# vyasakash231/gaussian_process_transportation

Measured on AMD Instinct MI355X. Metric: posterior (mean+var+Jacobian) preds/sec, N=8192 source pts, 3-D fp64, higher is better.
Workload: dtype f64; 1 GPU; N=8192 source pts, M=500000 queries per GPU per step, D=O=3, mean+var+Jacobian, RBF GP, fp64; queries_per_gpu=500000, mode=J

## Files before the change

gaussian_process_transportation_amd/csrc/gpt_kvar_i8.h:

```cpp
#pragma once
#include "gpt_common.h"
#include "gpt_dispatch.h"
#include "gpt_exp.h"
#include "gpt_plan_i8.h"

namespace gpt {

typedef int v4i __attribute__((ext_vector_type(4)));

constexpr int I8_TILE_STEPS = I8_ROWS / I8_KSTEP;
constexpr size_t I8_A_STEP = (size_t)8 * 4 * 64;
constexpr size_t I8_B_STEP = (size_t)8 * 64;
constexpr size_t I8_CHUNK = I8_TILE_STEPS * I8_B_STEP;
constexpr size_t I8_LDS_BYTES = 2 * I8_CHUNK * sizeof(v4i);
constexpr size_t I8_PARK_WORDS = var_i8_park_bytes() / 4;

#ifndef GPT_ABL_I8
#define GPT_ABL_I8 0
#endif
constexpr bool I8_ABL_A = GPT_ABL_I8 == 1 || GPT_ABL_I8 == 3 || GPT_ABL_I8 == 6;
constexpr bool I8_ABL_B = GPT_ABL_I8 == 2 || GPT_ABL_I8 == 3 || GPT_ABL_I8 == 6;
constexpr bool I8_ABL_NOGEN = GPT_ABL_I8 == 4;
constexpr bool I8_ABL_NORED = GPT_ABL_I8 == 5;
constexpr bool I8_ABL_NOLDS = GPT_ABL_I8 == 6;

struct I8Tab {
    float m[I8_NMOD], rm[I8_NMOD];
    float inv[I8_NMOD];
    float w[I8_NMOD][I8_NMOD];
};
constexpr int i8_balanced(int x, int m) { x %= m; if (x < 0) x += m; return x > (m - 1) / 2 ? x - m : x; }
constexpr I8Tab make_i8_tab() {
    I8Tab t{};
    for (int i = 0; i < I8_NMOD; ++i) {
        const int m = I8_MODULI[i];
        t.m[i] = (float)m; t.rm[i] = 1.0f / (float)m;
        int prod = 1;
        for (int l = 0; l < I8_NMOD; ++l) {
            t.w[l][i] = l < i ? (float)i8_balanced(prod, m) : 0.0f;
            if (l < i) prod = prod * I8_MODULI[l] % m;
        }
        int inv = 0;
        for (int x = 1; x < m; ++x) if (prod * x % m == 1) inv = x;
        t.inv[i] = (float)i8_balanced(inv, m);
    }
    return t;
}
static constexpr I8Tab I8_TAB = make_i8_tab();

__constant__ double c_i8_mod[I8_NMOD] = {256, 255, 253, 251, 247, 241, 239, 233, 229, 227, 223, 217, 211, 199};
__constant__ double c_i8_inv[I8_NMOD] = {1.0 / 256, 1.0 / 255, 1.0 / 253, 1.0 / 251, 1.0 / 247, 1.0 / 241, 1.0 / 239,
                                         1.0 / 233, 1.0 / 229, 1.0 / 227, 1.0 / 223, 1.0 / 217, 1.0 / 211, 1.0 / 199};
__constant__ double c_i8_hi[I8_NMOD] = {127, 127, 126, 125, 123, 120, 119, 116, 114, 113, 111, 108, 105, 99};
__constant__ double c_i8_lo[I8_NMOD] = {-128, -127, -126, -125, -123, -120, -119, -116, -114, -113, -111, -108, -105, -99};

static __device__ __forceinline__ int i8_residue(const double x, const double m, const double inv, const double hi, const double lo) {
    const double q = rint(x * inv);
    double r = fma(-q, m, x);
    r = r > hi ? r - m : r;
    r = r < lo ? r + m : r;
    return (int)r;
}
static __device__ __forceinline__ int i8_pack4(const int r0, const int r1, const int r2, const int r3) {
    return (int)((unsigned)(r0 & 255) | ((unsigned)(r1 & 255) << 8) | ((unsigned)(r2 & 255) << 16) | ((unsigned)r3 << 24));
}
static __device__ __forceinline__ void i8_store_planes(const double (&x)[16], v4i* __restrict__ dst, const size_t stride) {
#pragma unroll 1
    for (int j = 0; j < I8_NMOD; ++j) {
        const double m = c_i8_mod[j], inv = c_i8_inv[j], hi = c_i8_hi[j], lo = c_i8_lo[j];
        int r[16];
#pragma unroll
        for (int b = 0; b < 16; ++b) r[b] = i8_residue(x[b], m, inv, hi, lo);
        v4i o;
#pragma unroll
        for (int v = 0; v < 4; ++v) o[v] = i8_pack4(r[4 * v], r[4 * v + 1], r[4 * v + 2], r[4 * v + 3]);
        dst[(size_t)j * stride] = o;
    }
}

__global__ __launch_bounds__(256) void k_i8_rowmax(const double* __restrict__ Wf, unsigned long long* __restrict__ rowmax) {
    const int tile = blockIdx.x, g = blockIdx.y, th = threadIdx.x;
    int ib = 0;
    while ((ib + 1) * (ib + 2) / 2 <= tile) ++ib;
    const double* src = Wf + (size_t)tile * WT_TILE_DOUBLES + (size_t)g * 256 + th;
    double mx = 0.0;
    for (int k4 = 0; k4 < WT_K4; ++k4) mx = fmax(mx, fabs(src[(size_t)k4 * WT_STEP_DOUBLES]));
    const int q = th >> 7, lane = (th >> 1) & 63, pp = th & 1;
    const int row = ib * WT + 64 * g + 16 * (2 * q + pp) + (lane & 15);
    if (mx > 0.0) atomicMax(rowmax + row, (unsigned long long)__double_as_longlong(mx));
}
__global__ __launch_bounds__(256) void k_i8_rowscale(const unsigned long long* __restrict__ rowmax, int NP, int p, double* __restrict__ rowscale,
                                                     double* __restrict__ qscale) {
    const int i = blockIdx.x * 256 + threadIdx.x;
    if (i >= NP) return;
    const double mx = __longlong_as_double((long long)rowmax[i]);
    int e = 0;
    if (mx > 0.0) {
        int ex;
        const double f = frexp(mx, &ex);
        e = f == 0.5 ? ex - 1 : ex;
    }
    rowscale[i] = ldexp(1.0, e - p);
    qscale[i] = ldexp(1.0, p - e);
}
__global__ __launch_bounds__(256) void k_i8_planes(const double* __restrict__ Wf, const double* __restrict__ qscale, int ntiles, v4i* __restrict__ planes) {
    const int tile = blockIdx.x, g = blockIdx.y;
    int ib = 0;
    while ((ib + 1) * (ib + 2) / 2 <= tile) ++ib;
    const double* src = Wf + (size_t)tile * WT_TILE_DOUBLES;
    for (int u = threadIdx.x; u < I8_TILE_STEPS * 4 * 64; u += 256) {
        const int lane = u & 63, r = (u >> 6) & 3, s = u >> 8;
        const int lr = lane & 15, lk = lane >> 4;
        const double sc = qscale[ib * WT + 64 * g + 16 * r + lr];
        double x[16];
#pragma unroll
        for (int b = 0; b < 16; ++b) {
            const int col = 64 * s + 16 * lk + b;
            const int k4 = col >> 2, lkk = col & 3;
            x[b] = rint(src[((((size_t)k4 * 8 + g) * 2 + (r >> 1)) * 64 + lkk * 16 + lr) * 2 + (r & 1)] * sc);
        }
        v4i* dst = planes + ((((size_t)tile * I8_TILE_STEPS + s) * 8 + g) * 4 + r) * 64 + lane;
        i8_store_planes(x, dst, (size_t)ntiles * I8_TILE_STEPS * I8_A_STEP);
    }
}

static __device__ __forceinline__ double i8_garner(const float (&r)[I8_NMOD]) {
    float d[I8_NMOD];
    d[0] = r[0];
#pragma unroll
    for (int i = 1; i < I8_NMOD; ++i) {
        float s = 0.0f;
#pragma unroll
        for (int l = 0; l < i; ++l) s = fmaf(d[l], I8_TAB.w[l][i], s);
        float u = r[i] - s;
        u = fmaf(-rintf(u * I8_TAB.rm[i]), I8_TAB.m[i], u);
        const float v = u * I8_TAB.inv[i];
        d[i] = fmaf(-rintf(v * I8_TAB.rm[i]), I8_TAB.m[i], v);
    }
    double X = (double)d[I8_NMOD - 1];
#pragma unroll
    for (int i = I8_NMOD - 2; i >= 0; --i) X = fma(X, (double)I8_TAB.m[i], (double)d[i]);
    return X;
}

struct VarI8Args {
    const v4i* planes;
    const double* rowscale;
    const double* Xs;
    const double* Xq;
    int64_t M;
    double* slab;
    v4i* bimg;
    unsigned* park;
    double bq;
    double colscale;
    int ntiles;
};

template <int KT>
__global__ __launch_bounds__(512, 2) void k_var_i8(KernelParams p, VarI8PlanDev pl, VarI8Args a) {
    extern __shared__ __attribute__((aligned(16))) unsigned char i8_lds_raw[];
    v4i* const Bs = reinterpret_cast<v4i*>(i8_lds_raw);
    __shared__ double red[8][I8_COLS];
    __shared__ double Tt[256];
    const int tid = threadIdx.x, lane = tid & 63;
    const int w = __builtin_amdgcn_readfirstlane(tid >> 6);
    const int lc = lane & 15, lk = lane >> 4;
    const int g = (w < 4) ? w : (11 - w);
    const int nbi = pl.nbi, D = p.D;
    const int nst = p.NP / I8_KSTEP;
    if (tid < 256) Tt[tid] = g_exp2_table[tid];
    v4i* const bim = a.bimg + (size_t)blockIdx.x * ((size_t)I8_NMOD * nst * I8_B_STEP);
    unsigned* const pk = a.park + (size_t)blockIdx.x * I8_PARK_WORDS + tid;
    const size_t a_plane = (size_t)a.ntiles * I8_TILE_STEPS * I8_A_STEP;
    const v4i* const a_group = a.planes + (size_t)g * 256;
    const unsigned ulane = lane, utid = tid;
    constexpr double RS2 = 0.70710678118654752440;
    const double lnc = p.lnc;
    const int64_t n_rounds = pl.rnd_end - pl.rnd_begin;

    for (int64_t it = 0;; ++it) {
        int64_t cb; int ib_lo, ib_hi;
        if (it < n_rounds) {
            cb = (pl.rnd_begin + it) * pl.P + blockIdx.x; ib_lo = 0; ib_hi = nbi;
        } else {
            if (it > n_rounds || !pl.with_tail || pl.nparts <= 0) break;
            const int64_t c = blockIdx.x / pl.nparts;
            if (c >= pl.ncb - pl.nfull) break;
            const int q = blockIdx.x % pl.nparts;
            cb = pl.nfull + c; ib_lo = pl.bounds[q]; ib_hi = pl.bounds[q + 1];
        }
        __syncthreads();
        __builtin_amdgcn_fence(__ATOMIC_ACQ_REL, "workgroup");
        {
            const int64_t col = cb * I8_COLS + 16 * w + lc;
            const int64_t mm = col < a.M ? col : a.M - 1;
            const double* qp = a.Xq + mm * D;
            double q[3];
#pragma unroll
            for (int d = 0; d < 3; ++d) q[d] = qp[d < D ? d : 0] * ((d < D) ? p.inv_ls[d] * 0.70710678118654752440 : 0.0);
#pragma unroll 1
            for (int s = 0; s < (I8_ABL_NOGEN ? 0 : I8_TILE_STEPS * ib_hi); ++s) {
                const double* xp = a.Xs + (size_t)(I8_KSTEP * s + 16 * lk) * 4;
                double x[16];
#pragma unroll
                for (int b = 0; b < 16; ++b) {
                    const d4 xs = *reinterpret_cast<const d4*>(xp + 4 * b);
                    const double d0 = xs[0] * RS2 - q[0], d1 = xs[1] * RS2 - q[1], d2_ = xs[2] * RS2 - q[2];
                    double hh = d0 * d0;
                    hh = fma(d1, d1, hh);
                    hh = fma(d2_, d2_, hh);
                    x[b] = rint(kernel_tab<KT>(hh, lnc, Tt) * a.bq);
                }
                i8_store_planes(x, bim + ((size_t)s * 8 + w) * 64 + lane, (size_t)nst * I8_B_STEP);
            }
        }
        asm volatile("s_waitcnt vmcnt(0)" ::: "memory");
        __syncthreads();

        for (int ib = ib_hi - 1; ib >= ib_lo; --ib) {
            const int nmine = (g + 2) & ~1;
            const int lim = I8_TILE_STEPS * ib + nmine;
            const size_t tile0 = (size_t)ib * (ib + 1) / 2;
            auto a_ptr = [&](int j, int S) -> const v4i* {
                if (S >= lim) { S -= lim; ++j; }
                if (S >= lim) { S -= lim; ++j; }
                if (j >= I8_NMOD) { j = I8_NMOD - 1; S = lim - 1; }
                if (I8_ABL_A) S &= I8_TILE_STEPS - 1;
                return a_group + (size_t)j * a_plane + (tile0 * I8_TILE_STEPS + S) * I8_A_STEP;
            };
            {
                v4i t8[8];
#pragma unroll
                for (int i = 0; i < 8; ++i) t8[i] = bim[utid + 512 * i];
#pragma unroll
                for (int i = 0; i < 8; ++i) Bs[tid + 512 * i] = t8[i];
            }
            v4i ar[4][4];
#pragma unroll
            for (int i = 0; i < 4; ++i) {
                const v4i* ap = a_ptr(0, i);
#pragma unroll
                for (int r = 0; r < 4; ++r) ar[i][r] = ap[ulane + 64 * r];
            }
            __syncthreads();
            v4i acc[4][8];
#pragma unroll
            for (int r = 0; r < 4; ++r)
#pragma unroll
                for (int t = 0; t < 8; ++t) acc[r][t] = v4i{0, 0, 0, 0};
            int buf = 0;
            auto tile = [&](auto full_tag, const int nrun, const bool more_rt, const int j, const int S0, const v4i* nsrc) __attribute__((always_inline)) {
                constexpr bool FULL = decltype(full_tag)::value;
                const bool more = FULL || more_rt;
                if (I8_ABL_B) nsrc = bim;
                const v4i* bcur = Bs + (size_t)buf * I8_CHUNK + lane;
                v4i* bnext = Bs + (size_t)(buf ^ 1) * I8_CHUNK + tid;
                v4i st[3];
                v4i bq[3];
                if (I8_ABL_NOLDS) bq[0] = bq[1] = bq[2] = bcur[0];
#pragma unroll
                for (int s = 0; s < I8_TILE_STEPS; ++s) {
                    const bool run = FULL || s < nrun;
                    if (more && s == 0) st[0] = nsrc[utid];
                    if (more && s + 1 < I8_TILE_STEPS) st[(s + 1) % 3] = nsrc[utid + 512 * (s + 1)];
                    __builtin_amdgcn_sched_barrier(0);
                    if (run) {
                        if (!I8_ABL_NOLDS && (s == 0 || !FULL)) {
                            bq[(8 * s) % 3] = bcur[(8 * s) * 64];
                            bq[(8 * s + 1) % 3] = bcur[(8 * s + 1) * 64];
                        }
#pragma unroll
                        for (int t = 0; t < 8; ++t) {
                            const int u = 8 * s + t;
                            if (!I8_ABL_NOLDS && (t + 2 < 8 || (FULL && s + 1 < I8_TILE_STEPS))) bq[(u + 2) % 3] = bcur[(u + 2) * 64];
                            __builtin_amdgcn_sched_barrier(0);
#pragma unroll
                            for (int r = 0; r < 4; ++r)
                                acc[r][t] = __builtin_amdgcn_mfma_i32_16x16x64_i8(ar[s & 3][r], bq[u % 3], acc[r][t], 0, 0, 0);
                            __builtin_amdgcn_sched_barrier(0);
                        }
                    }
                    __builtin_amdgcn_sched_barrier(0);
                    if (more && s > 0) bnext[512 * (s - 1)] = st[(s - 1) % 3];
                    if (run) {
                        const v4i* ap = a_ptr(j, S0 + s + 4);
#pragma unroll
                        for (int r = 0; r < 4; ++r) ar[s & 3][r] = ap[ulane + 64 * r];
                    }
                    __builtin_amdgcn_sched_barrier(0);
                }
                if (more) bnext[512 * (I8_TILE_STEPS - 1)] = st[(I8_TILE_STEPS - 1) % 3];
                __syncthreads();
                buf ^= 1;
            };
#pragma unroll 1
            for (int j = 0; j < I8_NMOD; ++j) {
#pragma unroll 1
                for (int kb = 0; kb < ib; ++kb)
                    tile(Bool<true>{}, I8_TILE_STEPS, true, j, kb * I8_TILE_STEPS, bim + ((size_t)j * nst + (kb + 1) * I8_TILE_STEPS) * I8_B_STEP);
                tile(Bool<false>{}, nmine, j + 1 < I8_NMOD, j, ib * I8_TILE_STEPS, bim + (size_t)(j + 1) * nst * I8_B_STEP);
                if (I8_ABL_NORED) {
#pragma unroll
                    for (int r = 0; r < 4; ++r)
#pragma unroll
                        for (int t = 0; t < 8; ++t) asm volatile("" : "+v"(acc[r][t]));
                } else {
                    const double m = c_i8_mod[j], inv = c_i8_inv[j], hi = c_i8_hi[j], lo = c_i8_lo[j];
#pragma unroll
                    for (int r = 0; r < 4; ++r)
#pragma unroll
                        for (int t = 0; t < 8; ++t) {
                            int rr[4];
#pragma unroll
                            for (int e = 0; e < 4; ++e) rr[e] = i8_residue((double)acc[r][t][e], m, inv, hi, lo);
                            pk[(size_t)(j * 32 + r * 8 + t) * 512] = (unsigned)i8_pack4(rr[0], rr[1], rr[2], rr[3]);
                            acc[r][t] = v4i{0, 0, 0, 0};
                        }
                }
                const bool turn = (nmine & 2) != 0;
#pragma unroll
                for (int i = 0; i < 2; ++i)
#pragma unroll
                    for (int r = 0; r < 4; ++r) {
                        const v4i lo2 = ar[i][r], hi2 = ar[i + 2][r];
                        ar[i][r] = turn ? hi2 : lo2;
                        ar[i + 2][r] = turn ? lo2 : hi2;
                    }
            }
            asm volatile("s_waitcnt vmcnt(0)" ::: "memory");
#pragma unroll 1
            for (int t = 0; t < 8; ++t) {
                double ssq = 0.0;
#pragma unroll 1
                for (int r = 0; r < (I8_ABL_NORED ? 0 : 4); ++r) {
                    unsigned wd[I8_NMOD];
#pragma unroll
                    for (int j = 0; j < I8_NMOD; ++j) wd[j] = pk[(size_t)(j * 32 + r * 8 + t) * 512];
                    const d4 rs = *reinterpret_cast<const d4*>(a.rowscale + (size_t)ib * I8_ROWS + 64 * g + 16 * r + 4 * lk);
#pragma unroll
                    for (int e = 0; e < 4; ++e) {
                        float res[I8_NMOD];
#pragma unroll
                        for (int j = 0; j < I8_NMOD; ++j) res[j] = (float)((int)(wd[j] << (24 - 8 * e)) >> 24);
                        const double v = i8_garner(res) * rs[e] * a.colscale;
                        ssq = fma(v, v, ssq);
                    }
                }
                ssq += __shfl_xor(ssq, 16);
                ssq += __shfl_xor(ssq, 32);
                if (lk == 0) red[w][16 * t + lc] = ssq;
            }
            __syncthreads();
            if (tid < I8_COLS) {
                double v = 0.0;
#pragma unroll
                for (int ww = 0; ww < 8; ++ww) v += red[ww][tid];
                a.slab[((size_t)cb * nbi + ib) * I8_COLS + tid] = v;
            }
        }
    }
}

__global__ __launch_bounds__(I8_COLS) void k_var_i8_finalize(KernelParams p, int nbi, const double* __restrict__ slab, int64_t M,
                                                             const double* __restrict__ hdr, double* __restrict__ var) {
    const int64_t cb = blockIdx.x, m = cb * I8_COLS + threadIdx.x;
    if (m >= M) return;
    double s2 = 0.0;
    for (int ib = 0; ib < nbi; ++ib) s2 += slab[((size_t)cb * nbi + ib) * I8_COLS + threadIdx.x];
    const double v = hdr[16] + p.noise - s2;
    var[m] = v < 0.0 ? 0.0 : v;
}

}
```

Baseline: 1.734 million predictions/s.

## Compute int8 residues via byte-dot-product and float bias tricks; fold Garner inverse

Replaces the fp64 rint/fma residue reduction used for operand plane generation and accumulator reduction with an integer path. Values are split into bytes through a double-bias bit trick and reduced mod m with udot4 against precomputed powers of 256. A float magic-bias rounding then yields the balanced residue. Garner reconstruction folds the inverse into the weights, saving one reduction per digit, and new ablation switches are added. The aim is to cut scarce fp64 ALU work, at the cost of relying on bias-range assumptions that must hold for correctness.

Result: faster. 1.892 million predictions/s, median of 6 (+9.1%).

```diff
diff --git a/gaussian_process_transportation_amd/csrc/gpt_kvar_i8.h b/gaussian_process_transportation_amd/csrc/gpt_kvar_i8.h
--- a/gaussian_process_transportation_amd/csrc/gpt_kvar_i8.h
+++ b/gaussian_process_transportation_amd/csrc/gpt_kvar_i8.h
@@ -3,6 +3,7 @@
 #include "gpt_dispatch.h"
 #include "gpt_exp.h"
 #include "gpt_plan_i8.h"
+#include "gpt_residue_i8.h"
 
 namespace gpt {
 
@@ -23,58 +24,25 @@
 constexpr bool I8_ABL_NOGEN = GPT_ABL_I8 == 4;
 constexpr bool I8_ABL_NORED = GPT_ABL_I8 == 5;
 constexpr bool I8_ABL_NOLDS = GPT_ABL_I8 == 6;
-
-struct I8Tab {
-    float m[I8_NMOD], rm[I8_NMOD];
-    float inv[I8_NMOD];
-    float w[I8_NMOD][I8_NMOD];
-};
-constexpr int i8_balanced(int x, int m) { x %= m; if (x < 0) x += m; return x > (m - 1) / 2 ? x - m : x; }
-constexpr I8Tab make_i8_tab() {
-    I8Tab t{};
-    for (int i = 0; i < I8_NMOD; ++i) {
-        const int m = I8_MODULI[i];
-        t.m[i] = (float)m; t.rm[i] = 1.0f / (float)m;
-        int prod = 1;
-        for (int l = 0; l < I8_NMOD; ++l) {
-            t.w[l][i] = l < i ? (float)i8_balanced(prod, m) : 0.0f;
-            if (l < i) prod = prod * I8_MODULI[l] % m;
-        }
-        int inv = 0;
-        for (int x = 1; x < m; ++x) if (prod * x % m == 1) inv = x;
-        t.inv[i] = (float)i8_balanced(inv, m);
-    }
-    return t;
-}
-static constexpr I8Tab I8_TAB = make_i8_tab();
-
-__constant__ double c_i8_mod[I8_NMOD] = {256, 255, 253, 251, 247, 241, 239, 233, 229, 227, 223, 217, 211, 199};
-__constant__ double c_i8_inv[I8_NMOD] = {1.0 / 256, 1.0 / 255, 1.0 / 253, 1.0 / 251, 1.0 / 247, 1.0 / 241, 1.0 / 239,
-                                         1.0 / 233, 1.0 / 229, 1.0 / 227, 1.0 / 223, 1.0 / 217, 1.0 / 211, 1.0 / 199};
-__constant__ double c_i8_hi[I8_NMOD] = {127, 127, 126, 125, 123, 120, 119, 116, 114, 113, 111, 108, 105, 99};
-__constant__ double c_i8_lo[I8_NMOD] = {-128, -127, -126, -125, -123, -120, -119, -116, -114, -113, -111, -108, -105, -99};
-
-static __device__ __forceinline__ int i8_residue(const double x, const double m, const double inv, const double hi, const double lo) {
-    const double q = rint(x * inv);
-    double r = fma(-q, m, x);
-    r = r > hi ? r - m : r;
-    r = r < lo ? r + m : r;
-    return (int)r;
-}
-static __device__ __forceinline__ int i8_pack4(const int r0, const int r1, const int r2, const int r3) {
-    return (int)((unsigned)(r0 & 255) | ((unsigned)(r1 & 255) << 8) | ((unsigned)(r2 & 255) << 16) | ((unsigned)r3 << 24));
-}
+constexpr bool I8_ABL_NOPLANEST = GPT_ABL_I8 == 7;
+constexpr bool I8_ABL_NOPARK = GPT_ABL_I8 == 8;
+
+template <bool STORE = true>
 static __device__ __forceinline__ void i8_store_planes(const double (&x)[16], v4i* __restrict__ dst, const size_t stride) {
+    uint32_t lo[16], hi[16];
+#pragma unroll
+    for (int b = 0; b < 16; ++b) i8_operand_split(x[b], lo[b], hi[b]);
+    const I8ResTab& T = i8_res_tab();
 #pragma unroll 1
     for (int j = 0; j < I8_NMOD; ++j) {
-        const double m = c_i8_mod[j], inv = c_i8_inv[j], hi = c_i8_hi[j], lo = c_i8_lo[j];
-        int r[16];
-#pragma unroll
-        for (int b = 0; b < 16; ++b) r[b] = i8_residue(x[b], m, inv, hi, lo);
+        uint32_t r[16];
+#pragma unroll
+        for (int b = 0; b < 16; ++b) r[b] = i8_operand_bits(lo[b], hi[b], T, j);
         v4i o;
 #pragma unroll
-        for (int v = 0; v < 4; ++v) o[v] = i8_pack4(r[4 * v], r[4 * v + 1], r[4 * v + 2], r[4 * v + 3]);
-        dst[(size_t)j * stride] = o;
+        for (int v = 0; v < 4; ++v) o[v] = (int)i8_pack_bits(r[4 * v], r[4 * v + 1], r[4 * v + 2], r[4 * v + 3]);
+        if (STORE) dst[(size_t)j * stride] = o;
+        else asm volatile("" ::"v"(o));
     }
 }
 
@@ -126,20 +94,10 @@
 
 static __device__ __forceinline__ double i8_garner(const float (&r)[I8_NMOD]) {
     float d[I8_NMOD];
-    d[0] = r[0];
-#pragma unroll
-    for (int i = 1; i < I8_NMOD; ++i) {
-        float s = 0.0f;
-#pragma unroll
-        for (int l = 0; l < i; ++l) s = fmaf(d[l], I8_TAB.w[l][i], s);
-        float u = r[i] - s;
-        u = fmaf(-rintf(u * I8_TAB.rm[i]), I8_TAB.m[i], u);
-        const float v = u * I8_TAB.inv[i];
-        d[i] = fmaf(-rintf(v * I8_TAB.rm[i]), I8_TAB.m[i], v);
-    }
+    i8_garner_digits(r, d);
     double X = (double)d[I8_NMOD - 1];
 #pragma unroll
-    for (int i = I8_NMOD - 2; i >= 0; --i) X = fma(X, (double)I8_TAB.m[i], (double)d[i]);
+    for (int i = I8_NMOD - 2; i >= 0; --i) X = fma(X, (double)I8_GARNER.m[i], (double)d[i]);
     return X;
 }
 
@@ -212,7 +170,7 @@
                     hh = fma(d2_, d2_, hh);
                     x[b] = rint(kernel_tab<KT>(hh, lnc, Tt) * a.bq);
                 }
-                i8_store_planes(x, bim + ((size_t)s * 8 + w) * 64 + lane, (size_t)nst * I8_B_STEP);
+                i8_store_planes<!I8_ABL_NOPLANEST>(x, bim + ((size_t)s * 8 + w) * 64 + lane, (size_t)nst * I8_B_STEP);
             }
         }
         asm volatile("s_waitcnt vmcnt(0)" ::: "memory");
@@ -306,15 +264,17 @@
 #pragma unroll
                         for (int t = 0; t < 8; ++t) asm volatile("" : "+v"(acc[r][t]));
                 } else {
-                    const double m = c_i8_mod[j], inv = c_i8_inv[j], hi = c_i8_hi[j], lo = c_i8_lo[j];
+                    const I8ResTab& T = i8_res_tab();
 #pragma unroll
                     for (int r = 0; r < 4; ++r)
 #pragma unroll
                         for (int t = 0; t < 8; ++t) {
-                            int rr[4];
-#pragma unroll
-                            for (int e = 0; e < 4; ++e) rr[e] = i8_residue((double)acc[r][t][e], m, inv, hi, lo);
-                            pk[(size_t)(j * 32 + r * 8 + t) * 512] = (unsigned)i8_pack4(rr[0], rr[1], rr[2], rr[3]);
+                            uint32_t rr[4];
+#pragma unroll
+                            for (int e = 0; e < 4; ++e) rr[e] = i8_acc_bits(acc[r][t][e], T, j);
+                            const unsigned pw = i8_pack_bits(rr[0], rr[1], rr[2], rr[3]);
+                            if (I8_ABL_NOPARK) asm volatile("" ::"v"(pw));
+                            else pk[(size_t)(j * 32 + r * 8 + t) * 512] = pw;
                             acc[r][t] = v4i{0, 0, 0, 0};
                         }
                 }
@@ -336,7 +296,10 @@
                 for (int r = 0; r < (I8_ABL_NORED ? 0 : 4); ++r) {
                     unsigned wd[I8_NMOD];
 #pragma unroll
-                    for (int j = 0; j < I8_NMOD; ++j) wd[j] = pk[(size_t)(j * 32 + r * 8 + t) * 512];
+                    for (int j = 0; j < I8_NMOD; ++j) {
+                        if (I8_ABL_NOPARK) asm volatile("" : "=v"(wd[j]));
+                        else wd[j] = pk[(size_t)(j * 32 + r * 8 + t) * 512];
+                    }
                     const d4 rs = *reinterpret_cast<const d4*>(a.rowscale + (size_t)ib * I8_ROWS + 64 * g + 16 * r + 4 * lk);
 #pragma unroll
                     for (int e = 0; e < 4; ++e) {
diff --git a/gaussian_process_transportation_amd/csrc/gpt_residue_i8.h b/gaussian_process_transportation_amd/csrc/gpt_residue_i8.h
--- /dev/null
+++ b/gaussian_process_transportation_amd/csrc/gpt_residue_i8.h
@@ -0,0 +1,136 @@
+#pragma once
+#include <cstdint>
+
+#include "gpt_plan_i8.h"
+
+#if defined(__HIPCC__)
+#define GPT_RES_HD __host__ __device__
+#else
+#define GPT_RES_HD
+#endif
+
+namespace gpt {
+
+constexpr double I8_OPERAND_BIAS = 6755399441055744.0;
+constexpr int I8_ACC_BIAS = 1 << 30;
+constexpr uint32_t I8_FBIAS_BITS = 0x4B400000u;
+constexpr float I8_FBIAS = 12582912.0f;
+
+struct I8ResTab {
+    float m[I8_NMOD], rm[I8_NMOD];
+    uint32_t op_lo[I8_NMOD];
+    uint32_t op_hi[I8_NMOD];
+    uint32_t op_k[I8_NMOD];
+    uint32_t acc_k[I8_NMOD];
+};
+constexpr I8ResTab make_i8_res_tab() {
+    I8ResTab t{};
+    for (int j = 0; j < I8_NMOD; ++j) {
+        const int m = I8_MODULI[j];
+        t.m[j] = (float)m; t.rm[j] = 1.0f / (float)m;
+        uint32_t pw = 1 % m, lo = 0, hi = 0;
+        for (int i = 0; i < 7; ++i) {
+            if (i < 4) lo |= pw << (8 * i); else hi |= pw << (8 * (i - 4));
+            pw = pw * 256 % m;
+        }
+        t.op_lo[j] = lo; t.op_hi[j] = hi;
+        uint32_t p2 = 1 % m, k30 = 0;
+        for (int i = 0; i < 51; ++i) {
+            if (i == 30) k30 = (m - p2) % m;
+            p2 = p2 * 2 % m;
+        }
+        t.acc_k[j] = I8_FBIAS_BITS + k30; t.op_k[j] = I8_FBIAS_BITS + (m - p2) % m;
+    }
+    return t;
+}
+static constexpr I8ResTab I8_RES_HOST = make_i8_res_tab();
+#if defined(__HIPCC__)
+static __constant__ I8ResTab c_i8_res = make_i8_res_tab();
+#endif
+GPT_RES_HD inline const I8ResTab& i8_res_tab() {
+#if defined(__HIP_DEVICE_COMPILE__)
+    return c_i8_res;
+#else
+    return I8_RES_HOST;
+#endif
+}
+
+GPT_RES_HD inline uint32_t i8_udot4(const uint32_t a, const uint32_t b, const uint32_t acc) {
+#if defined(__HIP_DEVICE_COMPILE__)
+    return __builtin_amdgcn_udot4(a, b, acc, false);
+#else
+    uint32_t s = acc;
+    for (int i = 0; i < 4; ++i) s += ((a >> (8 * i)) & 255u) * ((b >> (8 * i)) & 255u);
+    return s;
+#endif
+}
+
+GPT_RES_HD inline uint32_t i8_balanced_bits(const uint32_t tbits, const float m, const float rm) {
+    float tb;
+    __builtin_memcpy(&tb, &tbits, 4);
+    const float tf = tb - I8_FBIAS;
+    const float rb = __builtin_fmaf(-__builtin_rintf(tf * rm), m, tb);
+    uint32_t o;
+    __builtin_memcpy(&o, &rb, 4);
+    return o;
+}
+GPT_RES_HD inline int i8_bits_int(const uint32_t rbits) { return (int)(rbits & 0x7FFFFFu) - 0x400000; }
+GPT_RES_HD inline int i8_bits_byte(const uint32_t rbits) { return (int)(int8_t)(uint8_t)(rbits & 255u); }
+GPT_RES_HD inline uint32_t i8_pack_bits(const uint32_t r0, const uint32_t r1, const uint32_t r2, const uint32_t r3) {
+    return (r0 & 255u) | ((r1 & 255u) << 8) | ((r2 & 255u) << 16) | (r3 << 24);
+}
+
+GPT_RES_HD inline void i8_operand_split(const double x, uint32_t& lo, uint32_t& hi) {
+    const double y = x + I8_OPERAND_BIAS;
+    uint64_t b;
+    __builtin_memcpy(&b, &y, 8);
+    lo = (uint32_t)b; hi = (uint32_t)(b >> 32) & 0xFFFFFu;
+}
+GPT_RES_HD inline uint32_t i8_operand_bits(const uint32_t lo, const uint32_t hi, const I8ResTab& T, const int j) {
+    return i8_balanced_bits(i8_udot4(lo, T.op_lo[j], i8_udot4(hi, T.op_hi[j], T.op_k[j])), T.m[j], T.rm[j]);
+}
+GPT_RES_HD inline uint32_t i8_acc_bits(const int32_t a, const I8ResTab& T, const int j) {
+    return i8_balanced_bits(i8_udot4((uint32_t)a + (uint32_t)I8_ACC_BIAS, T.op_lo[j], T.acc_k[j]), T.m[j], T.rm[j]);
+}
+
+struct I8GarnerTab {
+    float m[I8_NMOD], rm[I8_NMOD];
+    float inv[I8_NMOD];
+    float nwi[I8_NMOD][I8_NMOD];
+};
+constexpr int i8_balanced(int x, int m) { x %= m; if (x < 0) x += m; return x > (m - 1) / 2 ? x - m : x; }
+constexpr I8GarnerTab make_i8_garner_tab() {
+    I8GarnerTab t{};
+    for (int i = 0; i < I8_NMOD; ++i) {
+        const int m = I8_MODULI[i];
+        t.m[i] = (float)m; t.rm[i] = 1.0f / (float)m;
+        int prod = 1, w[I8_NMOD] = {};
+        for (int l = 0; l < i; ++l) {
+            w[l] = prod;
+            prod = prod * I8_MODULI[l] % m;
+        }
+        int inv = 0;
+        for (int x = 1; x < m; ++x) if (prod * x % m == 1) inv = x;
+        t.inv[i] = (float)i8_balanced(inv, m);
+        for (int l = 0; l < I8_NMOD; ++l) t.nwi[l][i] = l < i ? (float)-i8_balanced(w[l] * inv, m) : 0.0f;
+    }
+    return t;
+}
+static constexpr I8GarnerTab I8_GARNER = make_i8_garner_tab();
+
+GPT_RES_HD inline void i8_garner_digits(const float (&r)[I8_NMOD], float (&d)[I8_NMOD]) {
+    d[0] = r[0];
+#if defined(__HIP_DEVICE_COMPILE__)
+#pragma unroll
+#endif
+    for (int i = 1; i < I8_NMOD; ++i) {
+        float v = r[i] * I8_GARNER.inv[i];
+#if defined(__HIP_DEVICE_COMPILE__)
+#pragma unroll
+#endif
+        for (int l = 0; l < i; ++l) v = __builtin_fmaf(d[l], I8_GARNER.nwi[l][i], v);
+        d[i] = __builtin_fmaf(-__builtin_rintf(v * I8_GARNER.rm[i]), I8_GARNER.m[i], v);
+    }
+}
+
+}
```
